# scaleoutsystems/fedn

Hardware: AMD Instinct MI355X
Metric: aggregated params/sec (device-resident) — FedAvg 64-client reduce, 100M fp32 (higher is better)
Workload: dtype f32

## Files before the change

### fedn_amd/csrc/fedagg.hip

```cpp

#include <hip/hip_runtime.h>
#include <hip/hip_fp16.h>

#include <cmath>
#include <cstdarg>
#include <cstdint>
#include <cstdio>
#include <algorithm>
#include <atomic>
#include <cstring>
#include <type_traits>
#include <vector>

#include "../../include/fedagg.h"
#ifdef FEDAGG_PROBES
#include "../../include/fedagg_probe.h"
#endif

namespace {

thread_local char g_err[512] = "";
thread_local const char* g_kernel = "";

int fail(int code, const char* fmt, ...) {
// ... 456 lines not shown
                fold_strip<CP, E>(x[s], yv, n, N, r);
            }
        }
#pragma unroll
        for (int s = 0; s < S; ++s) {
            X xo[E];
#pragma unroll
            for (int e = 0; e < E; ++e) xo[e] = narrow<X, V>(x[s][e]);
            strip_store<X, E>(agg + (strip0 + s * kBlock) * E, xo);
        }
    } else {
        k_fedavg_tail<Y, X, CP, E, S, INIT, INT_FIRST>(agg, tab, K, P, strip0);
    }
}

template <class CP>
struct LaneTable {
    uint64_t p;
    typename CP::S n, N;
    double r;
    __device__ __forceinline__ explicit LaneTable(const ClientTable<typename CP::S>& tab) {
        const int lane = threadIdx.x & 63;
        p = reinterpret_cast<uint64_t>(tab.ptr[lane]);
        n = tab.n[lane];
        N = tab.N[lane];
        r = tab.r[lane];
    }
    template <typename T>
    __device__ __forceinline__ static T rl(T v, int k) {
        static_assert(sizeof(T) == 4 || sizeof(T) == 8, "readlane of 4/8-byte values");
        if constexpr (sizeof(T) == 4) {
            int i;
            __builtin_memcpy(&i, &v, 4);
            i = __builtin_amdgcn_readlane(i, k);
            __builtin_memcpy(&v, &i, 4);
            return v;
        } else {
            int i[2];
            __builtin_memcpy(i, &v, 8);
            i[0] = __builtin_amdgcn_readlane(i[0], k);
            i[1] = __builtin_amdgcn_readlane(i[1], k);
            __builtin_memcpy(&v, i, 8);
            return v;
        }
    }
};

[[maybe_unused]] __device__ __forceinline__ bool in_write_window(uint32_t period, uint32_t win_w) {
    const uint32_t t = (uint32_t)__builtin_amdgcn_s_memrealtime();
    uint32_t r;
    if ((period & (period - 1)) == 0) {
        r = t & (period - 1);
    } else {
        const uint32_t recip = 0xFFFFFFFFu / period;
        r = t - __umulhi(t, recip) * period;
        if (r >= period) r -= period;
    }
    return r < win_w;
}
[[maybe_unused]] __device__ __forceinline__ void wait_write_window(uint32_t period, uint32_t win_w) {
    for (int n = 0; n < (1 << 18) && !in_write_window(period, win_w); ++n) __builtin_amdgcn_s_sleep(1);
}
[[maybe_unused]] __device__ __forceinline__ void wait_read_window(uint32_t period, uint32_t win_w) {
    for (int n = 0; n < (1 << 18) && in_write_window(period, win_w); ++n) __builtin_amdgcn_s_sleep(1);
}


template <int MAP>
__device__ __forceinline__ int64_t map_tile(int64_t t, int64_t ntiles) {
    if constexpr (MAP > 0) {
        const int64_t g = ntiles / (8 * MAP);
        if (t < 8 * MAP * g) {
            const int64_t j = t / 8;
            t = (j / MAP) * (8 * MAP) + (t % 8) * MAP + (j % MAP);
        }
    }
    return t;
}

template <typename Y, typename X, class CP, int E, int S, bool INIT, bool INT_FIRST, bool NT, bool LT, int BLK, int NTS,
          int MAP, bool WIN = false>
__device__ __forceinline__ void fedavg_pipe_body(X* __restrict__ agg, const ClientTable<typename CP::S>& tab, const int K,
                                                 const int64_t P, const uint32_t period = 0, const uint32_t win_w = 0,
                                                 const int win_mode = 0) {
    using V = typename CP::V;
    const LaneTable<CP> lt(tab);
    const int64_t ntiles = ((P + E - 1) / E + (int64_t)BLK * S - 1) / ((int64_t)BLK * S);
    for (int64_t t = blockIdx.x; t < ntiles; t += gridDim.x) {
        const int64_t tile = map_tile<MAP>(t, ntiles);
        const int64_t strip0 = tile * (BLK * S) + threadIdx.x;
        if ((strip0 + (int64_t)(S - 1) * BLK) * E + E > P) {
            k_fedavg_tail<Y, X, CP, E, S, INIT, INT_FIRST, BLK>(agg, tab, K, P, strip0);
            continue;
        }
        if constexpr (WIN) {
            if (win_mode >= 1) wait_read_window(period, win_w);
        }
        V x[S][E];
        int k = 0;
#pragma unroll
        for (int s = 0; s < S; ++s)
            k = strip_start<Y, X, CP, E, INIT, INT_FIRST, NT>(x[s], agg, tab, (strip0 + s * BLK) * E, E);
        auto load = [&](int kk, Y (&y)[S][E]) {
            const Y* yp = LT ? reinterpret_cast<const Y*>(LaneTable<CP>::rl(lt.p, kk)) : static_cast<const Y*>(tab.ptr[kk]);
#pragma unroll
            for (int s = 0; s < S; ++s) strip_load<Y, E, NT>(yp + (strip0 + s * BLK) * E, y[s]);
        };
        auto fold = [&](int kk, const Y (&y)[S][E]) {
            const typename CP::S n = LT ? LaneTable<CP>::rl(lt.n, kk) : tab.n[kk];
            const typename CP::S N = LT ? LaneTable<CP>::rl(lt.N, kk) : tab.N[kk];
            const double r = LT ? LaneTable<CP>::rl(lt.r, kk) : tab.r[kk];
#pragma unroll
            for (int s = 0; s < S; ++s) {
                V yv[E];
#pragma unroll
                for (int e = 0; e < E; ++e) yv[e] = widen<Y, V>(y[s][e]);
                fold_strip<CP, E>(x[s], yv, n, N, r);
            }
        };
        Y a[S][E], b[S][E];
        if (k < K) load(k, a);
        while (k + 1 < K) {
            if constexpr (WIN) {
                if (win_mode >= 2) wait_read_window(period, win_w);
            }
            load(k + 1, b);
            fold(k, a);
            if (k + 2 < K) load(k + 2, a);
            fold(k + 1, b);
            k += 2;
        }
        if (k < K) fold(k, a);
        if constexpr (WIN) wait_write_window(period, win_w);
#pragma unroll
        for (int s = 0; s < S; ++s) {
            X xo[E];
#pragma unroll
            for (int e = 0; e < E; ++e) xo[e] = narrow<X, V>(x[s][e]);
            if constexpr (is_nostore<CP>::value) {
                if (__float_as_uint(x[s][0]) != 0xFFFFFFFFu) continue;
            }
            strip_store<X, E, NTS>(agg + (strip0 + s * BLK) * E, xo);
        }
    }
}

template <typename Y, typename X, class CP, int E, int S, bool INIT, bool INT_FIRST, bool NT, bool LT, int BLK = kBlock,
          int NTS = 0, int MAP = 0>
__global__ void __launch_bounds__(BLK)
k_fedavg_pipe(X* __restrict__ agg, const ClientTable<typename CP::S> tab, const int K, const int64_t P) {
    fedavg_pipe_body<Y, X, CP, E, S, INIT, INT_FIRST, NT, LT, BLK, NTS, MAP>(agg, tab, K, P);
}

template <typename Y, typename X, class CP, int E, int S, bool INIT, bool INT_FIRST, bool NT, bool LT, int BLK, int NTS,
          int MAP>
__global__ void __launch_bounds__(BLK)
k_fedavg_pipe_win(X* __restrict__ agg, const ClientTable<typename CP::S> tab, const int K, const int64_t P,
                  const uint32_t period, const uint32_t win_w, const int win_mode) {
    fedavg_pipe_body<Y, X, CP, E, S, INIT, INT_FIRST, NT, LT, BLK, NTS, MAP, true>(agg, tab, K, P, period, win_w, win_mode);
}

struct OptScalars {
    double lr, b1, b2, tau, tau2, c1, c2, nc2;
    float b1f, c1f, c2f;
    float b1h, c1h, c2h;
    int opt;
};

struct OptBuffers {
    const void* old;
    void* pg;
    const void* m_in;
    void* m_out;
    const void* v_in;
    void* v_out;
    void* out;
    int m_in_f64;
    int m_out_f64;
    int v_in_f32;
    int v_out_f32;
    int out_f32;
};

template <class PG> __device__ __forceinline__ double mul_pg(double a, double c, float cf, float ch);
template <> __device__ __forceinline__ double mul_pg<CF32>(double a, double, float cf, float) { return (double)((float)a * cf); }
template <> __device__ __forceinline__ double mul_pg<CF64>(double a, double c, float, float) { return a * c; }
template <> __device__ __forceinline__ double mul_pg<CF16>(double a, double, float, float ch) {
    return (double)CF16::rh((float)a * ch);
}

template <class PG> __device__ __forceinline__ typename PG::V pg_sub(typename PG::V y, typename PG::V o) { return y - o; }
template <> __device__ __forceinline__ float pg_sub<CF16>(float y, float o) { return CF16::rh(y - o); }
template <class PG> __device__ __forceinline__ typename PG::V pg_sq(typename PG::V v) { return (typename PG::V)(v * v); }
template <> __device__ __forceinline__ float pg_sq<CF16>(float v) { return CF16::rh(v * v); }

__device__ __forceinline__ double np_sign(double d) {
    return d > 0.0 ? 1.0 : (d < 0.0 ? -1.0 : (d == 0.0 ? 0.0 : d));
}

template <int E, bool SNT = false>
__device__ __forceinline__ void opt_load_state(const OptBuffers& b, const OptScalars& s, int64_t i0, int rem,
                                               double (&mi)[E], double (&v)[E]) {
    const bool full = rem == E;
    if (b.m_in_f64 == 0) {
        float mf[E];
        const float* mp = static_cast<const float*>(b.m_in) + i0;
        if (full) strip_load<float, E, SNT>(mp, mf);
        else
            for (int e = 0; e < E; ++e) mf[e] = e < rem ? mp[e] : 0.f;
#pragma unroll
        for (int e = 0; e < E; ++e) mi[e] = (double)mf[e];
    } else if (b.m_in_f64 == 1) {
        const double* mp = static_cast<const double*>(b.m_in) + i0;
        if (full) strip_load<double, E, SNT>(mp, mi);
        else
            for (int e = 0; e < E; ++e) mi[e] = e < rem ? mp[e] : 0.0;
    } else if (b.m_in_f64 == 2) {
        f16 mh[E];
        const f16* mp = static_cast<const f16*>(b.m_in) + i0;
        if (full) strip_load<f16, E, SNT>(mp, mh);
        else
            for (int e = 0; e < E; ++e) mh[e] = e < rem ? mp[e] : f16{0};
#pragma unroll
        for (int e = 0; e < E; ++e) mi[e] = (double)f16_to_f32(mh[e].bits);
    }
    if (b.v_in && b.v_in_f32) {
        float vf[E];
        const float* vp = static_cast<const float*>(b.v_in) + i0;
        if (full) strip_load<float, E, SNT>(vp, vf);
        else
            for (int e = 0; e < E; ++e) vf[e] = e < rem ? vp[e] : 0.f;
#pragma unroll
        for (int e = 0; e < E; ++e) v[e] = (double)vf[e];
    } else if (b.v_in) {
        const double* vp = static_cast<const double*>(b.v_in) + i0;
        if (full) strip_load<double, E, SNT>(vp, v);
        else
            for (int e = 0; e < E; ++e) v[e] = e < rem ? vp[e] : 0.0;
    } else {
#pragma unroll
        for (int e = 0; e < E; ++e) v[e] = s.tau2;
    }
}

template <class PG, int E, bool NOST = false, int OSM = 0>
__device__ __forceinline__ void opt_apply(const OptBuffers& b, const OptScalars& s, const typename PG::V (&pg)[E],
                                          const typename PG::V (&ov)[E], const double (&mi)[E], double (&v)[E],
                                          int64_t i0, int rem) {
    using V = typename PG::V;
    constexpr bool PG32 = std::is_same<PG, CF32>::value;
    const bool full = rem == E;
    constexpr bool PG64 = std::is_same<PG, CF64>::value;
    double m[E];
    if (b.m_in_f64 < 0) {
#pragma unroll
        for (int e = 0; e < E; ++e) m[e] = mul_pg<PG>((double)pg[e], s.c1, s.c1f, s.c1h);
    } else {
        if (b.m_in_f64 == 1) {
#pragma unroll
            for (int e = 0; e < E; ++e) m[e] = mi[e] * s.b1 + mul_pg<PG>((double)pg[e], s.c1, s.c1f, s.c1h);
        } else if (b.m_in_f64 == 0) {
#pragma unroll
            for (int e = 0; e < E; ++e) {
                const float a = (float)mi[e] * s.b1f;
                const double pm = mul_pg<PG>((double)pg[e], s.c1, s.c1f, s.c1h);
                if constexpr (PG64) m[e] = (double)a + pm;
                else m[e] = (double)(a + (float)pm);
            }
        } else {
#pragma unroll
            for (int e = 0; e < E; ++e) {
                const float a = CF16::rh((float)mi[e] * s.b1h);
                const double pm = mul_pg<PG>((double)pg[e], s.c1, s.c1f, s.c1h);
                if constexpr (PG64) m[e] = (double)a + pm;
                else if constexpr (PG32) m[e] = (double)(a + (float)pm);
                else m[e] = (double)CF16::rh(a + (float)pm);
            }
        }
    }
    double o[E];
#pragma unroll
    for (int e = 0; e < E; ++e) {
        const V pv = pg[e];
        const double p = (double)pg_sq<PG>(pv);
        if (s.opt == FA_ADAM) {
            v[e] = v[e] * s.b2 + mul_pg<PG>(p, s.c2, s.c2f, s.c2h);
        } else if (s.opt == FA_YOGI) {
            const double sg = np_sign(v[e] - p);
            v[e] = v[e] + (sg * p) * s.nc2;
        } else {
            v[e] = v[e] + p;
        }
        const double sv = __builtin_sqrt(v[e]) + s.tau;
        const double t = m[e] / sv;
        o[e] = (double)ov[e] + t * s.lr;
    }
    if constexpr (NOST) {
        if (__double_as_longlong(o[0]) != 0x7FF4DEADBEEF0001LL) return;
    }
    if (full) {
        if (b.v_out_f32) {
            float vf[E];
#pragma unroll
            for (int e = 0; e < E; ++e) vf[e] = (float)v[e];
            strip_store<float, E, OSM>(static_cast<float*>(b.v_out) + i0, vf);
        } else {
            strip_store<double, E, OSM>(static_cast<double*>(b.v_out) + i0, v);
        }
        if (b.out_f32) {
            float of[E];
#pragma unroll
            for (int e = 0; e < E; ++e) of[e] = (float)o[e];
// ... 558 lines not shown
        if constexpr (std::is_same<TO, f16>::value && std::is_integral<TI>::value)
            out[i] = f16{f32_to_f16((float)in[j])};
        else if constexpr (std::is_same<TO, f16>::value && std::is_same<TI, float>::value)
            out[i] = f16{f32_to_f16(in[j])};
        else if constexpr (std::is_same<TO, float>::value && std::is_same<TI, double>::value)
            out[i] = (float)in[j];
        else
            out[i] = widen<TI, TO>(in[j]);
    }
}

constexpr int kPushWords = 4;

__global__ void __launch_bounds__(kBlock) k_push(PushTable t, int nd, const u32x4* __restrict__ src, int64_t n16) {
    const int64_t stride = (int64_t)gridDim.x * kBlock * kPushWords;
    for (int64_t base = (int64_t)blockIdx.x * kBlock * kPushWords + threadIdx.x; base < n16; base += stride) {
        u32x4 v[kPushWords];
#pragma unroll
        for (int j = 0; j < kPushWords; ++j) {
            const int64_t i = base + (int64_t)j * kBlock;
            if (i < n16) v[j] = __builtin_nontemporal_load(src + i);
        }
        for (int d = 0; d < nd; ++d) {
            u32x4* __restrict__ o = t.dst[d];
#pragma unroll
            for (int j = 0; j < kPushWords; ++j) {
                const int64_t i = base + (int64_t)j * kBlock;
                if (i < n16) __builtin_nontemporal_store(v[j], o + i);
            }
        }
    }
}

__global__ void k_push_tail(PushTable t, int nd, const uint8_t* __restrict__ src, int64_t off, int rem) {
    const int b = threadIdx.x;
    if (b < rem)
        for (int d = 0; d < nd; ++d) reinterpret_cast<uint8_t*>(t.dst[d])[off + b] = src[off + b];
}

#ifdef FEDAGG_PROBES
__global__ void __launch_bounds__(kBlock) k_stream_copy(u32x4* __restrict__ dst, const u32x4* __restrict__ src, int64_t n16) {
    const int64_t i = (int64_t)blockIdx.x * kBlock + threadIdx.x;
    if (i < n16) dst[i] = __builtin_nontemporal_load(src + i);
}

constexpr int kReadPerLane = 16;
template <int RPL>
__global__ void __launch_bounds__(kBlock) k_stream_read(const u32x4* __restrict__ src, int64_t n16, u32x4* __restrict__ sink) {
    const int64_t base = (int64_t)blockIdx.x * kBlock * RPL + threadIdx.x;
    u32x4 acc = {0, 0, 0, 0};
#pragma unroll
    for (int j = 0; j < RPL; ++j) {
        const int64_t i = base + (int64_t)j * kBlock;
        if (i < n16) acc ^= __builtin_nontemporal_load(src + i);
    }
    __shared__ u32x4 red[kBlock];
    red[threadIdx.x] = acc;
    __syncthreads();
    if (threadIdx.x == 0) {
        u32x4 r = red[0];
        for (int t = 1; t < kBlock; ++t) r ^= red[t];
        sink[blockIdx.x] = r;
    }
}
#endif

bool aligned16(const void* p) { return (reinterpret_cast<uintptr_t>(p) & 15u) == 0; }

#ifdef FEDAGG_PROBES
struct FedAvgCfg {
    std::atomic<int> strips{4}, unroll{0}, lanetab{0}, grid_per_cu{0}, read_per_lane{16}, block_log{8},
        sum_nostore{0}, nt_store{1}, nt{0}, fastdiv{1}, fastdiv64{1}, narrow{1}, auto_geom{1}, opt_mix{0},
        opt_win_period{0}, opt_win_w{0}, opt_win_mode{0}, opt_win_prod{0}, avg_win_period{0}, avg_win_w{0},
        avg_win_mode{0};
};
FedAvgCfg g_cfg;
int cfg_fastdiv() { return g_cfg.fastdiv.load(std::memory_order_relaxed); }
int cfg_fastdiv64() { return g_cfg.fastdiv64.load(std::memory_order_relaxed); }
int cfg_grid_per_cu() { return g_cfg.grid_per_cu.load(std::memory_order_relaxed); }
#else
constexpr int cfg_fastdiv() { return 1; }
constexpr int cfg_fastdiv64() { return 1; }
constexpr int cfg_grid_per_cu() { return 0; }
#endif

template <typename S>
void fill_table(ClientTable<S>& t, const void* const* ptrs, const double* n, const double* N, int k0, int cnt) {
    for (int j = 0; j < cnt; ++j) {
        t.ptr[j] = ptrs[k0 + j];
        t.n[j] = (S)n[k0 + j];
        t.N[j] = (S)N[k0 + j];
        if constexpr (std::is_same<S, double>::value) {
            const double Nd = N[k0 + j], a = std::fabs(Nd);
            t.r[j] = (cfg_fastdiv64() && a >= 0x1p-60 && a <= 0x1p60) ? 1.0 / Nd : 0.0;
        } else {
            const float Nf = (float)N[k0 + j];
            t.r[j] = (cfg_fastdiv() && Nf != 0.0f && std::fabs(Nf) < 0x1p28f) ? 1.0 / (double)Nf : 0.0;
        }
    }
    for (int j = cnt; j < kMaxK; ++j) {
        t.ptr[j] = nullptr;
        t.n[j] = 0;
        t.N[j] = 0;
        t.r[j] = 0.0;
    }
}

float to_half_value(double v) { return (float)(_Float16)v; }

int64_t grid_for(int64_t P, int E) {
    const int64_t strips = (P + E - 1) / E;
    return (strips + kBlock - 1) / kBlock;
}

int device_cus() {
    int dev = 0, cus = 256;
    if (hipGetDevice(&dev) != hipSuccess ||
        hipDeviceGetAttribute(&cus, hipDeviceAttributeMultiprocessorCount, dev) != hipSuccess)
        cus = 256;
    return cus > 0 ? cus : 256;
}

struct StoreWindow {
    uint32_t period = 0, w = 0;
};
template <typename Y, typename OLD, class PG, bool NT>
StoreWindow opt_store_window(const OptBuffers& b, int K, int64_t P) {
    const bool state = b.m_in_f64 >= 0 || b.v_in;
    if (K < (state ? 32 : 8) || P < ((int64_t)1 << 24)) return {};
    static std::atomic<int> blocks_per_cu{-1};
    int nb = blocks_per_cu.load(std::memory_order_relaxed);
    if (nb < 0) {
        nb = 0;
        if (hipOccupancyMaxActiveBlocksPerMultiprocessor(&nb, k_fedopt_cw<Y, OLD, PG, NT>, kBlock, 0) != hipSuccess) nb = 0;
        blocks_per_cu.store(nb, std::memory_order_relaxed);
    }
    if (nb <= 0) return {};
    const double waves = (double)nb * (kBlock / 64) * device_cus();
    const double m_in = b.m_in_f64 == 1 ? 8 : b.m_in_f64 == 0 ? 4 : b.m_in_f64 < 0 ? 0 : 2;
    const double m_out = b.m_out_f64 == 1 ? 8 : b.m_out_f64 == 0 ? 4 : 2;
    const double rd = (double)K * sizeof(Y) + sizeof(OLD) + m_in + (b.v_in ? (b.v_in_f32 ? 4 : 8) : 0);
    const double wr = (b.out_f32 ? 4 : 8) + (b.v_out_f32 ? 4 : 8) + m_out;
    const double frac = wr / (rd + wr);
    if (frac > 0.25) return {};
    const double period = (state ? 0.35 : 0.65) * waves * 512.0 * (rd + wr) / 6.4e12 * 1e8;
    if (period < 1000 || period > 20000) return {};
    StoreWindow sw;
    sw.period = (uint32_t)period;
    sw.w = (uint32_t)(period * (state ? 0.15 : std::min(0.30, std::max(0.08, 1.15 * frac))));
    return sw;
}


struct AvgWindow {
    uint32_t period = 0, w = 0;
};
template <typename Y, typename X, class CP, int E, int S, bool NT, bool LT, int BLK, int NTS, int MAP>
AvgWindow avg_store_window(int K, int64_t P) {
    if (P < ((int64_t)1 << 24) || K < 2) return {};
    static std::atomic<int> blocks_per_cu{-1};
    int nb = blocks_per_cu.load(std::memory_order_relaxed);
    if (nb < 0) {
        nb = 0;
        if (hipOccupancyMaxActiveBlocksPerMultiprocessor(&nb, k_fedavg_pipe_win<Y, X, CP, E, S, true, false, NT, LT, BLK, NTS, MAP>,
                                                         BLK, 0) != hipSuccess)
            nb = 0;
        blocks_per_cu.store(nb, std::memory_order_relaxed);
    }
    if (nb <= 0) return {};
    if ((double)sizeof(X) / ((double)K * sizeof(Y) + sizeof(X)) > 0.15) return {};
    const double round_bytes = (double)nb * device_cus() * BLK * S * E * ((double)K * sizeof(Y) + sizeof(X));
    const double period = 0.45 * round_bytes / 6.4e12 * 1e8;
    if (period < 500 || period > 20000) return {};
    AvgWindow w;
    w.period = (uint32_t)period;
    w.w = (uint32_t)(0.15 * period);
    return w;
}

template <typename Y, typename X, class CP, int E, int S, bool NT, bool LT, int BLK = kBlock, int NTS = 0, int MAP = 0>
void launch_fedavg_pipe(X* a, const ClientTable<typename CP::S>& tab, int cnt, int64_t P, bool first, bool int_first,
                        hipStream_t st);
template <typename Y, typename X, class CP, int E, int S, int U, bool NT>
void launch_fedavg_geom(X* a, const ClientTable<typename CP::S>& tab, int cnt, int64_t P, bool first, bool int_first,
                        hipStream_t st);
template <typename Y, typename X, class CP, int E>
void launch_fedavg_small(X* a, const ClientTable<typename CP::S>& tab, int cnt, int64_t P, bool first, bool int_first,
                         hipStream_t st);
template <typename Y>
inline bool pipe_pays(int64_t P);

#ifdef FEDAGG_PROBES

void probe_avg_window(AvgWindow& w, int& mode) {
    const int period = g_cfg.avg_win_period;
    if (period < 0) w = AvgWindow{};
    else if (period > 0) {
        w = AvgWindow{(uint32_t)period, (uint32_t)g_cfg.avg_win_w.load()};
        mode = g_cfg.avg_win_mode.load();
    }
}

template <typename Y, typename X, class CP, int E, int S, bool NT, bool LT, int BLK, int NTS, int MAP>
bool probe_avg_window_cont(X* a, const ClientTable<typename CP::S>& tab, int cnt, int64_t P, bool first, bool int_first,
                           dim3 grid, hipStream_t st) {
    if constexpr (std::is_same<CP, CF32>::value && std::is_same<X, float>::value && S * E * (int)sizeof(Y) == 64 &&
                  BLK == kBlock && MAP == 0 && !LT && !NT && NTS == 1) {
        if (g_cfg.avg_win_period > 0 && !int_first && !first) {
            const uint32_t wl = (uint32_t)g_cfg.avg_win_period.load(), ww = (uint32_t)g_cfg.avg_win_w.load();
            g_kernel = "k_fedavg_pipe_win";
            hipLaunchKernelGGL((k_fedavg_pipe_win<Y, X, CP, E, S, false, false, NT, LT, BLK, NTS, MAP>), grid, dim3(BLK), 0, st, a, tab,
                               cnt, P, wl, ww, g_cfg.avg_win_mode.load());
            return true;
        }
    }
    return false;
}

template <typename Y, typename X, class CP, int E>
bool probe_fedavg_geometry(X* a, const ClientTable<typename CP::S>& tab, int cnt, int64_t P, bool first, bool int_first,
                           hipStream_t st) {
    const int block_log = g_cfg.block_log, strips = g_cfg.strips, unroll = g_cfg.unroll, nt = g_cfg.nt;
    const int lanetab = g_cfg.lanetab, nt_store = g_cfg.nt_store;
    const int key = (block_log == 9 ? 20000 : block_log == 10 ? 30000 : 0) + lanetab * 10000 + strips * 100 +
                    unroll * 2 + nt;
    constexpr bool narrowable = sizeof(Y) < sizeof(X) && E % 2 == 0;
    if (key == 4 * 100 + 0 && nt_store == 1) {
        if (g_cfg.auto_geom && (g_cfg.narrow || !narrowable)) return false;
        if (g_cfg.auto_geom && !pipe_pays<Y>(P)) {
            launch_fedavg_small<Y, X, CP, E>(a, tab, cnt, P, first, int_first, st);
            return true;
        }
        if constexpr (narrowable) {
            if (g_cfg.narrow) {
                launch_fedavg_pipe<Y, X, CP, E / 2, 8, false, false, kBlock, 1>(a, tab, cnt, P, first, int_first, st);
                return true;
            }
        }
    }
    switch (key) {
#define FA_GEOM(S_, U_, NT_) \
    case S_ * 100 + U_ * 2 + NT_: launch_fedavg_geom<Y, X, CP, E, S_, U_, NT_>(a, tab, cnt, P, first, int_first, st); return true;
#define FA_PIPE(KEY_, ...) \
    case KEY_: launch_fedavg_pipe<Y, X, CP, E, __VA_ARGS__>(a, tab, cnt, P, first, int_first, st); return true;
        FA_GEOM(1, 4, 0) FA_GEOM(1, 8, 0) FA_GEOM(1, 16, 0) FA_GEOM(2, 4, 0) FA_GEOM(2, 8, 0) FA_GEOM(2, 16, 0)
        FA_GEOM(4, 1, 0) FA_GEOM(4, 2, 0) FA_GEOM(4, 4, 0) FA_GEOM(8, 1, 0) FA_GEOM(8, 2, 0) FA_GEOM(16, 1, 0)
        FA_GEOM(1, 8, 1) FA_GEOM(4, 2, 1) FA_GEOM(8, 1, 1)
        FA_PIPE(2 * 100 + 0, 2, false, false)
        case 4 * 100 + 0:
            if (nt_store == 1) launch_fedavg_pipe<Y, X, CP, E, 4, false, false, kBlock, 1>(a, tab, cnt, P, first, int_first, st);
            else if (nt_store == 2) launch_fedavg_pipe<Y, X, CP, E, 4, false, false, kBlock, 2>(a, tab, cnt, P, first, int_first, st);
            else launch_fedavg_pipe<Y, X, CP, E, 4, false, false>(a, tab, cnt, P, first, int_first, st);
            return true;
        FA_PIPE(8 * 100 + 0, 8, false, false)
        FA_PIPE(4 * 100 + 1, 4, true, false)
        FA_PIPE(20000 + 4 * 100 + 0, 4, false, false, 512)
        FA_PIPE(30000 + 4 * 100 + 0, 4, false, false, 1024)
        FA_PIPE(20000 + 8 * 100 + 0, 8, false, false, 512)
        FA_PIPE(30000 + 2 * 100 + 0, 2, false, false, 1024)
        FA_PIPE(10000 + 2 * 100 + 0, 2, false, true)
        FA_PIPE(10000 + 4 * 100 + 0, 4, false, true)
        FA_PIPE(10000 + 8 * 100 + 0, 8, false, true)
#undef FA_PIPE
#undef FA_GEOM
        default: break;
    }
    launch_fedavg_geom<Y, X, CP, E, 1, kUnroll, false>(a, tab, cnt, P, first, int_first, st);
    return true;
}

template <typename Y, typename OLD, class PG, bool NT>
bool probe_fedopt_launch(const OptBuffers& b, const OptScalars& s, const ClientTable<typename PG::S>& tab, int cnt, int64_t P,
                         bool first, bool final_, dim3 g4, hipStream_t st, int& rc) {
    constexpr bool probe_combo = std::is_same<Y, float>::value && (std::is_same<OLD, float>::value || std::is_same<OLD, double>::value);
    const int period = g_cfg.opt_win_period, prod = g_cfg.opt_win_prod;
    if constexpr (probe_combo) {
        if (first && final_ && period > 0 && !prod) {
            if (b.m_out_f64 != 1) {
                rc = fail(FA_EINVAL, "fa_tune OPT_WIN probe: fp64 m out");
                return true;
            }
            hipLaunchKernelGGL((k_fedopt_mixw<Y, OLD, typename PG::S, NT>), g4, dim3(kBlock), 0, st, b, tab, cnt, P, (uint32_t)period,
                               (uint32_t)g_cfg.opt_win_w.load(), g_cfg.opt_win_mode.load());
            rc = check_launch("fa_fedopt_step: kernel launch");
            return true;
        }
        if (first && final_ && g_cfg.opt_mix) {
            hipLaunchKernelGGL((k_fedopt_mix<Y, OLD, typename PG::S, NT>), g4, dim3(kBlock), 0, st, b, tab, cnt, P);
            rc = check_launch("fa_fedopt_step: kernel launch");
            return true;
        }
    }
    if (!final_ && period > 0 && prod) {
        const uint32_t w = (uint32_t)g_cfg.opt_win_w.load();
        if (first)
            hipLaunchKernelGGL((k_fedopt_cwp<Y, OLD, PG, true, NT>), g4, dim3(kBlock), 0, st, b, s, tab, cnt, P, (uint32_t)period, w);
        else
            hipLaunchKernelGGL((k_fedopt_cwp<Y, OLD, PG, false, NT>), g4, dim3(kBlock), 0, st, b, s, tab, cnt, P, (uint32_t)period, w);
        rc = check_launch("fa_fedopt_step: kernel launch");
        return true;
    }
    return false;
}

void probe_opt_window(StoreWindow& sw) {
    const int period = g_cfg.opt_win_period;
    if (period < 0) sw = StoreWindow{};
    else if (period > 0 && g_cfg.opt_win_prod) sw = StoreWindow{(uint32_t)period, (uint32_t)g_cfg.opt_win_w.load()};
}
#endif

template <typename Y, typename X, class CP, int E, int S, bool NT, bool LT, int BLK, int NTS, int MAP>
void launch_fedavg_pipe(X* a, const ClientTable<typename CP::S>& tab, int cnt, int64_t P, bool first, bool int_first,
                        hipStream_t st) {
    g_kernel = "k_fedavg_pipe";
    const int64_t strips = (P + E - 1) / E;
    int64_t ntiles = (strips + (int64_t)BLK * S - 1) / ((int64_t)BLK * S);
    if (cfg_grid_per_cu() > 0) {
        if constexpr (MAP != 0) return launch_fedavg_pipe<Y, X, CP, E, S, NT, LT, BLK, NTS, 0>(a, tab, cnt, P, first, int_first, st);
        ntiles = std::min<int64_t>(ntiles, (int64_t)cfg_grid_per_cu() * device_cus());
    }
    const dim3 grid((unsigned)ntiles);
    if constexpr (std::is_same<CP, CF32>::value && std::is_same<X, float>::value &&
                  ((std::is_same<Y, float>::value && S * E == 16) || (std::is_same<Y, bf16>::value && S * E == 32)) &&
                  BLK == kBlock && MAP == 0 && !LT && !NT && NTS == 1) {
        if (first && !int_first && cfg_grid_per_cu() == 0) {
            AvgWindow w = avg_store_window<Y, X, CP, E, S, NT, LT, BLK, NTS, MAP>(cnt, P);
            int wm = 0;
#ifdef FEDAGG_PROBES
            probe_avg_window(w, wm);
#endif
            if (w.period) {
                g_kernel = "k_fedavg_pipe_win";
                hipLaunchKernelGGL((k_fedavg_pipe_win<Y, X, CP, E, S, true, false, NT, LT, BLK, NTS, MAP>), grid, dim3(BLK), 0, st, a,
                                   tab, cnt, P, w.period, w.w, wm);
                return;
            }
        }
    }
#ifdef FEDAGG_PROBES
    if (probe_avg_window_cont<Y, X, CP, E, S, NT, LT, BLK, NTS, MAP>(a, tab, cnt, P, first, int_first, grid, st)) return;
#endif
    if (first && int_first) {
        if constexpr (std::is_integral<Y>::value)
            hipLaunchKernelGGL((k_fedavg_pipe<Y, X, CP, E, S, true, true, NT, LT, BLK, NTS, MAP>), grid, dim3(BLK), 0, st, a, tab, cnt, P);
    } else if (first)
        hipLaunchKernelGGL((k_fedavg_pipe<Y, X, CP, E, S, true, false, NT, LT, BLK, NTS, MAP>), grid, dim3(BLK), 0, st, a, tab, cnt, P);
    else
        hipLaunchKernelGGL((k_fedavg_pipe<Y, X, CP, E, S, false, false, NT, LT, BLK, NTS, MAP>), grid, dim3(BLK), 0, st, a, tab, cnt, P);
}

template <typename Y, typename X, class CP, int E, int S, int U, bool NT>
void launch_fedavg_geom(X* a, const ClientTable<typename CP::S>& tab, int cnt, int64_t P, bool first, bool int_first,
                        hipStream_t st) {
    g_kernel = "k_fedavg";
    const int64_t strips = (P + E - 1) / E;
    const dim3 grid((unsigned)((strips + (int64_t)kBlock * S - 1) / ((int64_t)kBlock * S)));
    if (first && int_first) {
        if constexpr (std::is_integral<Y>::value)
            hipLaunchKernelGGL((k_fedavg<Y, X, CP, E, S, U, true, true, NT>), grid, dim3(kBlock), 0, st, a, tab, cnt, P);
    } else if (first)
        hipLaunchKernelGGL((k_fedavg<Y, X, CP, E, S, U, true, false, NT>), grid, dim3(kBlock), 0, st, a, tab, cnt, P);
    else
        hipLaunchKernelGGL((k_fedavg<Y, X, CP, E, S, U, false, false, NT>), grid, dim3(kBlock), 0, st, a, tab, cnt, P);
}

constexpr int64_t kPipeMinClientBytes = 160ll << 20;

template <typename Y>
inline bool pipe_pays(int64_t P) { return P * (int64_t)sizeof(Y) >= kPipeMinClientBytes; }

template <class CP> struct is_sf_rule : std::false_type {};
template <typename Y, typename X> struct is_sf_rule<CWSUM<Y, X>> : std::true_type {};
template <typename T_> struct is_sf_rule<CRUN<T_>> : std::true_type {};

template <typename Y, typename X, class CP, int E>
void launch_fedavg_default(X* a, const ClientTable<typename CP::S>& tab, int cnt, int64_t P, bool first, bool int_first,
                           hipStream_t st) {
    if (!pipe_pays<Y>(P)) return launch_fedavg_small<Y, X, CP, E>(a, tab, cnt, P, first, int_first, st);
    if constexpr (sizeof(Y) < sizeof(X) && E % 2 == 0)
        return launch_fedavg_pipe<Y, X, CP, E / 2, 8, false, false, kBlock, 1>(a, tab, cnt, P, first, int_first, st);
    else
        return launch_fedavg_pipe<Y, X, CP, E, 4, false, false, kBlock, 1>(a, tab, cnt, P, first, int_first, st);
}

template <typename Y, typename X, class CP, int E>
void launch_fedavg_vec(X* a, const ClientTable<typename CP::S>& tab, int cnt, int64_t P, bool first, bool int_first,
                       hipStream_t st) {
    constexpr bool tunable = (std::is_same<Y, float>::value || std::is_same<Y, bf16>::value) && std::is_same<X, float>::value &&
                             std::is_same<CP, CF32>::value;
    if constexpr (is_sf_rule<CP>::value) {
        if (!pipe_pays<Y>(P)) return launch_fedavg_small<Y, X, CP, E>(a, tab, cnt, P, first, int_first, st);
        launch_fedavg_pipe<Y, X, CP, E, 4, false, false>(a, tab, cnt, P, first, int_first, st);
        return;
    }
    if constexpr (tunable) {
#ifdef FEDAGG_PROBES
        if (probe_fedavg_geometry<Y, X, CP, E>(a, tab, cnt, P, first, int_first, st)) return;
#endif
        return launch_fedavg_default<Y, X, CP, E>(a, tab, cnt, P, first, int_first, st);
    }
    launch_fedavg_geom<Y, X, CP, E, 1, kUnroll, false>(a, tab, cnt, P, first, int_first, st);
}

template <typename Y, typename X, class CP, int E>
void launch_fedavg_small(X* a, const ClientTable<typename CP::S>& tab, int cnt, int64_t P, bool first, bool int_first,
                         hipStream_t st) {
    if (sizeof(Y) < 4 || cnt <= 8) launch_fedavg_geom<Y, X, CP, E, 1, 8, false>(a, tab, cnt, P, first, int_first, st);
    else launch_fedavg_geom<Y, X, CP, E, 1, 4, false>(a, tab, cnt, P, first, int_first, st);
}

template <typename Y, typename X, class CP>
int launch_fedavg(void* agg, const void* const* ups, const double* n, const double* N, int K, int64_t P,
                  int init, bool int_first, hipStream_t st) {
    constexpr int E16 = 16 / (int)sizeof(Y) > 0 ? 16 / (int)sizeof(Y) : 1;
    bool vec = aligned16(agg);
    for (int k = 0; k < K && vec; ++k) vec = aligned16(ups[k]);
    using S = typename CP::S;
    ClientTable<S> tab;
    int k0 = 0;
    bool first = init != 0;
    X* a = static_cast<X*>(agg);
    while (k0 < K) {
        const int cnt = (K - k0) < kMaxK ? (K - k0) : kMaxK;
        fill_table<S>(tab, ups, n, N, k0, cnt);
        if (std::is_same<CP, CF16>::value) {
            for (int j = 0; j < cnt; ++j) {
                tab.n[j] = (S)to_half_value(n[k0 + j]);
                tab.N[j] = (S)to_half_value(N[k0 + j]);
            }
        }
        if (vec) launch_fedavg_vec<Y, X, CP, E16>(a, tab, cnt, P, first, int_first, st);
        else launch_fedavg_geom<Y, X, CP, 1, 1, kUnroll, false>(a, tab, cnt, P, first, int_first, st);
        int rc = check_launch("fa_fedavg_fold: kernel launch");
        if (rc) return rc;
        first = false;
        k0 += cnt;
    }
    return FA_OK;
}

template <typename Y, typename OLD, class PG, int E, bool NT>
int launch_fedopt_one(const OptBuffers& b, const OptScalars& s, const ClientTable<typename PG::S>& tab, int cnt,
                      int64_t P, bool first, bool final_, hipStream_t st) {
    g_kernel = E == 4 ? "k_fedopt_c" : "k_fedopt";
    const dim3 grid((unsigned)grid_for(P, E));
    if constexpr (E == 4) {
        const dim3 g4((unsigned)((P + 4 * 512 - 1) / (4 * 512)));
#ifdef FEDAGG_PROBES
        int prc = FA_OK;
        if (probe_fedopt_launch<Y, OLD, PG, NT>(b, s, tab, cnt, P, first, final_, g4, st, prc)) return prc;
#endif
        if (first && final_) {
            StoreWindow sw = opt_store_window<Y, OLD, PG, NT>(b, cnt, P);
#ifdef FEDAGG_PROBES
            probe_opt_window(sw);
#endif
            if (sw.period) {
                g_kernel = "k_fedopt_cw";
                hipLaunchKernelGGL((k_fedopt_cw<Y, OLD, PG, NT>), g4, dim3(kBlock), 0, st, b, s, tab, cnt, P, sw.period, sw.w);
                return check_launch("fa_fedopt_step: kernel launch");
            }
        }
        if (first && final_) hipLaunchKernelGGL((k_fedopt_c<Y, OLD, PG, true, true, NT, 1, 4>), g4, dim3(kBlock), 0, st, b, s, tab, cnt, P);
        else if (first) hipLaunchKernelGGL((k_fedopt_c<Y, OLD, PG, true, false, NT, 1, 4>), g4, dim3(kBlock), 0, st, b, s, tab, cnt, P);
        else if (final_) hipLaunchKernelGGL((k_fedopt_c<Y, OLD, PG, false, true, NT, 1, 4>), g4, dim3(kBlock), 0, st, b, s, tab, cnt, P);
        else hipLaunchKernelGGL((k_fedopt_c<Y, OLD, PG, false, false, NT, 1, 4>), g4, dim3(kBlock), 0, st, b, s, tab, cnt, P);
    } else {
        if (first && final_) hipLaunchKernelGGL((k_fedopt<Y, OLD, PG, E, true, true, NT>), grid, dim3(kBlock), 0, st, b, s, tab, cnt, P);
        else if (first) hipLaunchKernelGGL((k_fedopt<Y, OLD, PG, E, true, false, NT>), grid, dim3(kBlock), 0, st, b, s, tab, cnt, P);
        else if (final_) hipLaunchKernelGGL((k_fedopt<Y, OLD, PG, E, false, true, NT>), grid, dim3(kBlock), 0, st, b, s, tab, cnt, P);
        else hipLaunchKernelGGL((k_fedopt<Y, OLD, PG, E, false, false, NT>), grid, dim3(kBlock), 0, st, b, s, tab, cnt, P);
    }
    return check_launch("fa_fedopt_step: kernel launch");
}

template <typename Y, typename OLD, class PG>
int launch_fedopt(const OptBuffers& b, const OptScalars& s, const void* const* ups, const double* n, const double* N,
                  int K, int64_t P, int flags, hipStream_t st) {
    bool vec = aligned16(b.old) && aligned16(b.pg) && aligned16(b.m_in) && aligned16(b.m_out) && aligned16(b.v_in) &&
               aligned16(b.v_out) && aligned16(b.out);
    for (int k = 0; k < K && vec; ++k) vec = aligned16(ups[k]);
    using S = typename PG::S;
    ClientTable<S> tab;
    bool first = (flags & FA_PG_FIRST) != 0;
// ... 575 lines not shown
    if (reinterpret_cast<uintptr_t>(src) % 16) return fail(FA_EINVAL, "fa_push: source not 16-B aligned");
    hipStream_t st = static_cast<hipStream_t>(stream);
    const int64_t n16 = bytes / 16;
    const int rem = (int)(bytes % 16);
    if (n16 > 0) {
        const int64_t need = (n16 + (int64_t)kBlock * kPushWords - 1) / ((int64_t)kBlock * kPushWords);
        const int grid = (int)std::min<int64_t>(need, 512);
        hipLaunchKernelGGL(k_push, dim3(grid), dim3(kBlock), 0, st, t, ndst, static_cast<const u32x4*>(src), n16);
    }
    if (rem > 0)
        hipLaunchKernelGGL(k_push_tail, dim3(1), dim3(64), 0, st, t, ndst, static_cast<const uint8_t*>(src), n16 * 16,
                           rem);
    hipError_t e = hipGetLastError();
    if (e != hipSuccess) return fail(FA_EHIP, "fa_push: %s", hipGetErrorString(e));
    return launch_release(st, release_rec);
}

int fa_device_xccs(int dev, int* n) {
    g_err[0] = 0;
    if (!n) return fail(FA_EINVAL, "fa_device_xccs: null argument");
    return device_xccs(dev, n);
}

int fa_host_device_ptr(const void* host, void** dptr) {
    g_err[0] = 0;
    if (!host || !dptr) return fail(FA_EINVAL, "fa_host_device_ptr: null argument");
    void* d = nullptr;
    hipError_t e = hipHostGetDevicePointer(&d, const_cast<void*>(host), 0);
    if (e != hipSuccess) {
        (void)hipGetLastError();
        return fail(FA_EHIP, "fa_host_device_ptr: %s (not page-locked host memory?)", hipGetErrorString(e));
    }
    *dptr = d;
    return FA_OK;
}

int fa_host_register(void* p, int64_t bytes) {
    g_err[0] = 0;
    if (!p || bytes <= 0) return fail(FA_EINVAL, "fa_host_register: bad arguments");
    hipError_t e = hipHostRegister(p, (size_t)bytes, hipHostRegisterPortable);
    if (e != hipSuccess) return fail(FA_EHIP, "fa_host_register: %s", hipGetErrorString(e));
    return FA_OK;
}

int fa_host_unregister(void* p) {
    g_err[0] = 0;
    if (!p) return FA_OK;
    hipError_t e = hipHostUnregister(p);
    if (e != hipSuccess) return fail(FA_EHIP, "fa_host_unregister: %s", hipGetErrorString(e));
    return FA_OK;
}

int fa_peer_enable(int dev, int peer) {
    g_err[0] = 0;
    if (dev == peer) return FA_OK;
    int can = 0;
    hipError_t e = hipDeviceCanAccessPeer(&can, dev, peer);
    if (e != hipSuccess) return fail(FA_EHIP, "fa_peer_enable: hipDeviceCanAccessPeer: %s", hipGetErrorString(e));
    if (!can) return fail(FA_EHIP, "fa_peer_enable: device %d cannot access device %d", dev, peer);
    int cur = 0;
    (void)hipGetDevice(&cur);
    e = hipSetDevice(dev);
    if (e == hipSuccess) e = hipDeviceEnablePeerAccess(peer, 0);
    (void)hipSetDevice(cur);
    if (e == hipErrorPeerAccessAlreadyEnabled) {
        (void)hipGetLastError();
        return FA_OK;
    }
    if (e != hipSuccess) return fail(FA_EHIP, "fa_peer_enable(%d -> %d): %s", dev, peer, hipGetErrorString(e));
    return FA_OK;
}

#ifdef FEDAGG_PROBES
int fa_tune(int knob, int value) {
    g_err[0] = 0;
    switch (knob) {
        case FA_TUNE_STRIPS:
            if (value != 1 && value != 2 && value != 4 && value != 8 && value != 16)
                return fail(FA_EINVAL, "fa_tune: strips must be 1, 2, 4, 8 or 16");
            g_cfg.strips = value;
            return FA_OK;
        case FA_TUNE_UNROLL:
            if (value != 0 && value != 1 && value != 2 && value != 4 && value != 8 && value != 16)
                return fail(FA_EINVAL, "fa_tune: unroll must be 0 (pipelined), 1, 2, 4, 8 or 16");
            g_cfg.unroll = value;
            return FA_OK;
        case FA_TUNE_NT:
            g_cfg.nt = value ? 1 : 0;
            return FA_OK;
        case FA_TUNE_SUM_NOSTORE:
            g_cfg.sum_nostore = value != 0;
            return FA_OK;
        case FA_TUNE_NT_STORE:
            if (value < 0 || value > 2) return fail(FA_EINVAL, "fa_tune: store mode 0 (plain), 1 (nt) or 2 (sc1)");
            g_cfg.nt_store = value;
            return FA_OK;
        case FA_TUNE_BLOCK:
            if (value != 256 && value != 512 && value != 1024) return fail(FA_EINVAL, "fa_tune: block 256, 512 or 1024");
            g_cfg.block_log = value == 256 ? 8 : value == 512 ? 9 : 10;
            return FA_OK;
        case FA_TUNE_READ:
            if (value != 4 && value != 8 && value != 16) return fail(FA_EINVAL, "fa_tune: read probe depth 4, 8 or 16");
            g_cfg.read_per_lane = value;
            return FA_OK;
        case FA_TUNE_GRID:
            if (value < 0 || value > 64) return fail(FA_EINVAL, "fa_tune: grid blocks per CU must be 0..64");
            g_cfg.grid_per_cu = value;
            return FA_OK;
        case FA_TUNE_LANETAB:
            g_cfg.lanetab = value ? 1 : 0;
            return FA_OK;
        case FA_TUNE_FASTDIV:
            g_cfg.fastdiv = value ? 1 : 0;
            return FA_OK;
        case FA_TUNE_FASTDIV64:
            g_cfg.fastdiv64 = value ? 1 : 0;
            return FA_OK;
        case FA_TUNE_NARROW:
            g_cfg.narrow = value ? 1 : 0;
            return FA_OK;
        case FA_TUNE_AUTO_GEOM:
            g_cfg.auto_geom = value ? 1 : 0;
            return FA_OK;
        case FA_TUNE_OPT_MIX:
            g_cfg.opt_mix = value ? 1 : 0;
            return FA_OK;
        case FA_TUNE_OPT_WIN_PERIOD:
            if (value != 0 && value != -1 && (value < 64 || value > (1 << 24)))
                return fail(FA_EINVAL, "fa_tune: store-window period 64 .. 2^24 ticks of 10 ns (0 = the product's own, -1 = none)");
            g_cfg.opt_win_period = value;
            return FA_OK;
        case FA_TUNE_OPT_WIN_W:
            if (value < 0) return fail(FA_EINVAL, "fa_tune: store-window length in ticks >= 0");
            g_cfg.opt_win_w = value;
            return FA_OK;
        case FA_TUNE_OPT_WIN_MODE:
            if (value < 0 || value > 2) return fail(FA_EINVAL, "fa_tune: store-window mode 0, 1 or 2");
            g_cfg.opt_win_mode = value;
            return FA_OK;
        case FA_TUNE_OPT_WIN_PROD:
            if (value != 0 && value != 1) return fail(FA_EINVAL, "fa_tune: OPT_WIN_PROD 0 (pattern probe) or 1 (k_fedopt_cw)");
            g_cfg.opt_win_prod = value;
            return FA_OK;
        case FA_TUNE_AVG_WIN_PERIOD:
            if (value != 0 && value != -1 && (value < 64 || value > (1 << 24)))
                return fail(FA_EINVAL, "fa_tune: store-window period 64 .. 2^24 ticks of 10 ns (0 = the product's own, -1 = none)");
            g_cfg.avg_win_period = value;
            return FA_OK;
        case FA_TUNE_AVG_WIN_W:
            if (value < 0) return fail(FA_EINVAL, "fa_tune: store-window length in ticks >= 0");
            g_cfg.avg_win_w = value;
            return FA_OK;
        case FA_TUNE_AVG_WIN_MODE:
            if (value < 0 || value > 2) return fail(FA_EINVAL, "fa_tune: store-window mode 0, 1 or 2");
            g_cfg.avg_win_mode = value;
            return FA_OK;
        default:
            return fail(FA_EINVAL, "fa_tune: unknown knob %d", knob);
    }
}

int fa_stream_sum(float* out, const float* const* bufs, int K, int64_t P, void* stream) {
    g_err[0] = 0;
    if (K < 1 || K > kMaxK || P < 0 || !out || !bufs) return fail(FA_EINVAL, "fa_stream_sum: bad arguments");
    bool vec = aligned16(out);
    for (int k = 0; k < K; ++k) vec = vec && bufs[k] && aligned16(bufs[k]);
    if (!vec) return fail(FA_EINVAL, "fa_stream_sum: buffers must be 16-B aligned");
    ClientTable<float> tab;
    std::vector<double> ones(K, 1.0);
    fill_table<float>(tab, reinterpret_cast<const void* const*>(bufs), ones.data(), ones.data(), 0, K);
    if (g_cfg.sum_nostore)
        launch_fedavg_pipe<float, float, CADDNW, 4, 4, false, false>(out, tab, K, P, true, false, static_cast<hipStream_t>(stream));
    else if (g_cfg.nt_store == 1)
        launch_fedavg_pipe<float, float, CADD, 4, 4, false, false, kBlock, 1>(out, tab, K, P, true, false, static_cast<hipStream_t>(stream));
    else if (g_cfg.nt_store == 2)
        launch_fedavg_pipe<float, float, CADD, 4, 4, false, false, kBlock, 2>(out, tab, K, P, true, false, static_cast<hipStream_t>(stream));
    else
        launch_fedavg_pipe<float, float, CADD, 4, 4, false, false>(out, tab, K, P, true, false, static_cast<hipStream_t>(stream));
    return check_launch("fa_stream_sum");
}

int fa_stream_copy(void* dst, const void* src, int64_t bytes, void* stream) {
    g_err[0] = 0;
    if (bytes < 0 || (bytes & 15) || !aligned16(dst) || !aligned16(src))
        return fail(FA_EINVAL, "fa_stream_copy: bytes must be a multiple of 16 and buffers 16-B aligned");
    const int64_t n16 = bytes / 16;
    if (!n16) return FA_OK;
    hipLaunchKernelGGL(k_stream_copy, dim3((unsigned)((n16 + kBlock - 1) / kBlock)), dim3(kBlock), 0,
                       static_cast<hipStream_t>(stream), static_cast<u32x4*>(dst), static_cast<const u32x4*>(src), n16);
    return check_launch("fa_stream_copy");
}

int64_t fa_stream_read_blocks(int64_t bytes) {
    const int64_t n16 = bytes / 16;
    const int64_t per = (int64_t)kBlock * kReadPerLane;
    return (n16 + per - 1) / per;
}

int fa_stream_read(const void* src, int64_t bytes, void* sink, void* stream) {
    g_err[0] = 0;
    if (bytes < 0 || (bytes & 15) || !aligned16(src) || !aligned16(sink))
        return fail(FA_EINVAL, "fa_stream_read: bytes must be a multiple of 16 and buffers 16-B aligned");
    const int64_t blocks = fa_stream_read_blocks(bytes);
    if (!blocks) return FA_OK;
    const int64_t n16 = bytes / 16;
    const dim3 blk(kBlock);
    hipStream_t st = static_cast<hipStream_t>(stream);
    const u32x4* s4 = static_cast<const u32x4*>(src);
    u32x4* k4 = static_cast<u32x4*>(sink);
    switch (g_cfg.read_per_lane) {
        case 4: hipLaunchKernelGGL(k_stream_read<4>, dim3((unsigned)((n16 + kBlock * 4 - 1) / (kBlock * 4))), blk, 0, st, s4, n16, k4); break;
        case 8: hipLaunchKernelGGL(k_stream_read<8>, dim3((unsigned)((n16 + kBlock * 8 - 1) / (kBlock * 8))), blk, 0, st, s4, n16, k4); break;
        default: hipLaunchKernelGGL(k_stream_read<16>, dim3((unsigned)blocks), blk, 0, st, s4, n16, k4); break;
    }
    return check_launch("fa_stream_read");
}

#endif

}
```

### include/fedagg_probe.h

```cpp
#ifndef FEDAGG_PROBE_H
#define FEDAGG_PROBE_H

#include "fedagg.h"

#ifdef __cplusplus
extern "C" {
#endif

int fa_stream_copy(void* dst, const void* src, int64_t bytes, void* stream);
int fa_stream_sum(float* out, const float* const* bufs, int K, int64_t P, void* stream);

enum fa_tune_knob {
    FA_TUNE_STRIPS = 0 ,
    FA_TUNE_UNROLL = 1 ,
    FA_TUNE_NT = 2 ,
    FA_TUNE_FASTDIV = 3 ,
    FA_TUNE_LANETAB = 4 ,
    FA_TUNE_GRID = 5 ,
    FA_TUNE_READ = 6 ,
    FA_TUNE_BLOCK = 7 ,
    FA_TUNE_SUM_NOSTORE = 8 ,
    FA_TUNE_NT_STORE = 9 ,
    FA_TUNE_FASTDIV64 = 10 ,
    FA_TUNE_NARROW = 11 ,
    FA_TUNE_AUTO_GEOM = 12 ,
    FA_TUNE_OPT_MIX = 13 ,
    FA_TUNE_OPT_WIN_PERIOD = 14 ,
    FA_TUNE_OPT_WIN_W = 15 ,
    FA_TUNE_OPT_WIN_MODE = 16 ,
    FA_TUNE_AVG_WIN_PERIOD = 17 ,
    FA_TUNE_AVG_WIN_W = 18,
    FA_TUNE_AVG_WIN_MODE = 19,
    FA_TUNE_OPT_WIN_PROD = 20
};
int fa_tune(int knob, int value);
int64_t fa_stream_read_blocks(int64_t bytes);
int fa_stream_read(const void* src, int64_t bytes, void* sink, void* stream);

#ifdef __cplusplus
}
#endif

#endif
```

Before: 1497 billion.

## Park FedAvg results in LDS and flush them during timed write windows

```diff
diff --git a/fedn_amd/csrc/fedagg.hip b/fedn_amd/csrc/fedagg.hip
--- a/fedn_amd/csrc/fedagg.hip
+++ b/fedn_amd/csrc/fedagg.hip
@@ -632,12 +632,110 @@
     fedavg_pipe_body<Y, X, CP, E, S, INIT, INT_FIRST, NT, LT, BLK, NTS, MAP>(agg, tab, K, P);
 }
 
+template <typename Y, typename X, class CP, int E, int S, int BLK, int NTS>
+__device__ __forceinline__ void fedavg_park_body(X* __restrict__ agg, const ClientTable<typename CP::S>& tab, const int K,
+                                                 const int64_t P, const uint32_t period, const uint32_t win_w) {
+    using V = typename CP::V;
+    static_assert(E * sizeof(X) == 16, "one 16-B piece per strip");
+    __shared__ u32x4 park[S * BLK];
+    constexpr int64_t kTile = (int64_t)BLK * S * E;
+    const int64_t ntiles = (P + kTile - 1) / kTile, nfull = P / kTile;
+    V x[S][E];
+    Y a[S][E], b[S][E];
+    int64_t t = blockIdx.x, parked = -1;
+    int k = 0;
+    const uint32_t lane_y = threadIdx.x * (uint32_t)(E * sizeof(Y)), lane_x = threadIdx.x * (uint32_t)(E * sizeof(X));
+    auto load = [&](int64_t tt, int kk, Y (&y)[S][E]) {
+        const char* base = static_cast<const char*>(tab.ptr[kk]) + tt * (kTile * (int64_t)sizeof(Y));
+#pragma unroll
+        for (int s = 0; s < S; ++s)
+            strip_load<Y, E, false>(reinterpret_cast<const Y*>(base + (int64_t)s * BLK * E * sizeof(Y) + lane_y), y[s]);
+    };
+    auto flush = [&]() {
+        char* base = reinterpret_cast<char*>(agg) + parked * (kTile * (int64_t)sizeof(X));
+#pragma unroll
+        for (int s = 0; s < S; ++s) {
+            X xo[E];
+            const u32x4 w = park[s * BLK + threadIdx.x];
+            __builtin_memcpy(xo, &w, 16);
+            strip_store<X, E, NTS>(reinterpret_cast<X*>(base + (int64_t)s * BLK * E * sizeof(X) + lane_x), xo);
+        }
+        parked = -1;
+    };
+    auto consume = [&](const Y (&cur)[S][E]) {
+        if (k == 0) {
+#pragma unroll
+            for (int s = 0; s < S; ++s)
+#pragma unroll
+                for (int e = 0; e < E; ++e) x[s][e] = widen<Y, V>(cur[s][e]);
+        } else {
+            const typename CP::S n = tab.n[k], N = tab.N[k];
+            const double r = tab.r[k];
+#pragma unroll
+            for (int s = 0; s < S; ++s) {
+                V yv[E];
+#pragma unroll
+                for (int e = 0; e < E; ++e) yv[e] = widen<Y, V>(cur[s][e]);
+                fold_strip<CP, E>(x[s], yv, n, N, r);
+            }
+        }
+        if (k == K - 1) {
+            if (parked >= 0) {
+                wait_write_window(period, win_w);
+                flush();
+            }
+#pragma unroll
+            for (int s = 0; s < S; ++s) {
+                X xo[E];
+#pragma unroll
+                for (int e = 0; e < E; ++e) xo[e] = narrow<X, V>(x[s][e]);
+                u32x4 w;
+                __builtin_memcpy(&w, xo, 16);
+                park[s * BLK + threadIdx.x] = w;
+            }
+            parked = t;
+        } else if ((k & 1) && parked >= 0 && in_write_window(period, win_w)) {
+            flush();
+        }
+    };
+    auto step = [&](const Y (&cur)[S][E], Y (&nxt)[S][E]) -> bool {
+        int k2 = k + 1;
+        int64_t t2 = t;
+        if (k2 == K) {
+            k2 = 0;
+            t2 += gridDim.x;
+        }
+        if (t2 >= nfull) {
+            consume(cur);
+            return false;
+        }
+        load(t2, k2, nxt);
+        consume(cur);
+        t = t2;
+        k = k2;
+        return true;
+    };
+    if (t < nfull) {
+        load(t, 0, a);
+        while (step(a, b) && step(b, a)) {
+        }
+    }
+    if (parked >= 0) flush();
+    if (nfull < ntiles && nfull % gridDim.x == blockIdx.x)
+        k_fedavg_tail<Y, X, CP, E, S, true, false, BLK>(agg, tab, K, P, nfull * (BLK * S) + threadIdx.x);
+}
+
 template <typename Y, typename X, class CP, int E, int S, bool INIT, bool INT_FIRST, bool NT, bool LT, int BLK, int NTS,
-          int MAP>
+          int MAP, bool PARK = false>
 __global__ void __launch_bounds__(BLK)
 k_fedavg_pipe_win(X* __restrict__ agg, const ClientTable<typename CP::S> tab, const int K, const int64_t P,
                   const uint32_t period, const uint32_t win_w, const int win_mode) {
-    fedavg_pipe_body<Y, X, CP, E, S, INIT, INT_FIRST, NT, LT, BLK, NTS, MAP, true>(agg, tab, K, P, period, win_w, win_mode);
+    if constexpr (PARK) {
+        static_assert(INIT && !INT_FIRST && !NT && !LT && MAP == 0, "parked stores: first launches of the product geometry");
+        fedavg_park_body<Y, X, CP, E, S, BLK, NTS>(agg, tab, K, P, period, win_w);
+    } else {
+        fedavg_pipe_body<Y, X, CP, E, S, INIT, INT_FIRST, NT, LT, BLK, NTS, MAP, true>(agg, tab, K, P, period, win_w, win_mode);
+    }
 }
 
 struct OptScalars {
@@ -1502,8 +1600,29 @@
 }
 
 
+template <typename Y, typename X, class CP, int E, int S, bool NT, bool LT, int BLK, int NTS, int MAP>
+constexpr bool avg_park_geometry = std::is_same<CP, CF32>::value && std::is_same<X, float>::value &&
+                                   std::is_same<Y, float>::value && S * E == 16 && BLK == kBlock && MAP == 0 && !LT && !NT;
+
+constexpr int kAvgParkPerCu = 2;
+template <typename Y, typename X, class CP, int E, int S, bool NT, bool LT, int BLK, int NTS, int MAP>
+int64_t avg_park_grid(int64_t ntiles, int per_cu) {
+    static std::atomic<int> blocks_per_cu{-1};
+    int nb = blocks_per_cu.load(std::memory_order_relaxed);
+    if (nb < 0) {
+        nb = 0;
+        if (hipOccupancyMaxActiveBlocksPerMultiprocessor(
+                &nb, k_fedavg_pipe_win<Y, X, CP, E, S, true, false, NT, LT, BLK, NTS, MAP, true>, BLK, 0) != hipSuccess)
+            nb = 0;
+        blocks_per_cu.store(nb, std::memory_order_relaxed);
+    }
+    nb = per_cu > 0 ? per_cu : std::min(std::max(nb, 1), kAvgParkPerCu);
+    return std::max<int64_t>(1, std::min<int64_t>(ntiles, (int64_t)nb * device_cus()));
+}
+
 struct AvgWindow {
     uint32_t period = 0, w = 0;
+    int mode = 0;
 };
 template <typename Y, typename X, class CP, int E, int S, bool NT, bool LT, int BLK, int NTS, int MAP>
 AvgWindow avg_store_window(int K, int64_t P) {
@@ -1525,6 +1644,14 @@
     AvgWindow w;
     w.period = (uint32_t)period;
     w.w = (uint32_t)(0.15 * period);
+    if constexpr (avg_park_geometry<Y, X, CP, E, S, NT, LT, BLK, NTS, MAP>) {
+        const double pperiod = 0.7 * period / 0.45 * kAvgParkPerCu / nb;
+        if (K >= 48 && pperiod >= 500 && pperiod <= 20000) {
+            w.period = (uint32_t)pperiod;
+            w.w = (uint32_t)(0.08 * pperiod);
+            w.mode = 3;
+        }
+    }
     return w;
 }
 
@@ -1556,7 +1683,7 @@
                            dim3 grid, hipStream_t st) {
     if constexpr (std::is_same<CP, CF32>::value && std::is_same<X, float>::value && S * E * (int)sizeof(Y) == 64 &&
                   BLK == kBlock && MAP == 0 && !LT && !NT && NTS == 1) {
-        if (g_cfg.avg_win_period > 0 && !int_first && !first) {
+        if (g_cfg.avg_win_period > 0 && g_cfg.avg_win_mode != 3 && !int_first && !first) {
             const uint32_t wl = (uint32_t)g_cfg.avg_win_period.load(), ww = (uint32_t)g_cfg.avg_win_w.load();
             g_kernel = "k_fedavg_pipe_win";
             hipLaunchKernelGGL((k_fedavg_pipe_win<Y, X, CP, E, S, false, false, NT, LT, BLK, NTS, MAP>), grid, dim3(BLK), 0, st, a, tab,
@@ -1674,13 +1801,24 @@
     if constexpr (std::is_same<CP, CF32>::value && std::is_same<X, float>::value &&
                   ((std::is_same<Y, float>::value && S * E == 16) || (std::is_same<Y, bf16>::value && S * E == 32)) &&
                   BLK == kBlock && MAP == 0 && !LT && !NT && NTS == 1) {
-        if (first && !int_first && cfg_grid_per_cu() == 0) {
+        if (first && !int_first) {
             AvgWindow w = avg_store_window<Y, X, CP, E, S, NT, LT, BLK, NTS, MAP>(cnt, P);
-            int wm = 0;
+            int wm = w.mode;
 #ifdef FEDAGG_PROBES
             probe_avg_window(w, wm);
 #endif
-            if (w.period) {
+            if constexpr (avg_park_geometry<Y, X, CP, E, S, NT, LT, BLK, NTS, MAP>) {
+                if (w.period && wm == 3) {
+                    const int64_t all = (strips + (int64_t)BLK * S - 1) / ((int64_t)BLK * S);
+                    const dim3 pgrid((unsigned)avg_park_grid<Y, X, CP, E, S, NT, LT, BLK, NTS, MAP>(all, cfg_grid_per_cu()));
+                    g_kernel = "k_fedavg_pipe_win";
+                    hipLaunchKernelGGL((k_fedavg_pipe_win<Y, X, CP, E, S, true, false, NT, LT, BLK, NTS, MAP, true>), pgrid, dim3(BLK),
+                                       0, st, a, tab, cnt, P, w.period, w.w, wm);
+                    return;
+                }
+            }
+            if (wm == 3) wm = 0;
+            if (w.period && cfg_grid_per_cu() == 0) {
                 g_kernel = "k_fedavg_pipe_win";
                 hipLaunchKernelGGL((k_fedavg_pipe_win<Y, X, CP, E, S, true, false, NT, LT, BLK, NTS, MAP>), grid, dim3(BLK), 0, st, a,
                                    tab, cnt, P, w.period, w.w, wm);
@@ -2562,7 +2700,7 @@
             g_cfg.avg_win_w = value;
             return FA_OK;
         case FA_TUNE_AVG_WIN_MODE:
-            if (value < 0 || value > 2) return fail(FA_EINVAL, "fa_tune: store-window mode 0, 1 or 2");
+            if (value < 0 || value > 3) return fail(FA_EINVAL, "fa_tune: store-window mode 0, 1, 2 or 3 (parked)");
             g_cfg.avg_win_mode = value;
             return FA_OK;
         default:
diff --git a/include/fedagg_probe.h b/include/fedagg_probe.h
--- a/include/fedagg_probe.h
+++ b/include/fedagg_probe.h
@@ -30,7 +30,7 @@
     FA_TUNE_OPT_WIN_MODE = 16 ,
     FA_TUNE_AVG_WIN_PERIOD = 17 ,
     FA_TUNE_AVG_WIN_W = 18,
-    FA_TUNE_AVG_WIN_MODE = 19,
+    FA_TUNE_AVG_WIN_MODE = 19 ,
     FA_TUNE_OPT_WIN_PROD = 20
 };
 int fa_tune(int knob, int value);
```

Measured after the change: 1528 billion, median of 6. 1.02x the previous value.
